# labicon/dp-ilqr

Hardware: AMD Instinct MI355X
Metric: ilqr_subproblems_per_sec (higher is better)
Workload: dtype f64; 1 GPU; cfg2: batches of 1024 independent 5-agent DoubleIntDynamics4D iLQR sub-problems per GPU per step, T=50, scripts/analysis.py scenario distribution, tol=1e-3, n_lqr_iter=50; 2468 steps = 2527232 distinct seeds per GPU, window of 6144 in flight; 1 repetition(s) of the job on disjoint seeds, the median is reported; batch_per_gpu=1024, window=6144, n_x=20, n_u=10, horizon=50, parallelism=single GPU

## Files before the change

### dpilqr_amd/csrc/riccati_mfma.hpp

```cpp
#pragma once
#include <hip/hip_runtime.h>

#include <type_traits>

#include "tiles.hpp"
#include "wave_util.hpp"

namespace dpilqr {

typedef double v4d __attribute__((ext_vector_type(4)));

template <int N, int M, int FUSED = 0, bool HELP = false>
struct MfmaCfg {
    static constexpr int NM = N + M;
    static constexpr int NP = N + 1;
    static constexpr int MK = round_up(M, 4);
    static constexpr int LAB = round_up(NM, 2);
    static constexpr int LT = LAB;
    static constexpr int LP = round_up(NP, 2);
    static constexpr int LQ = LP;
    static constexpr int LG = round_up(M + NP, 2);
    static constexpr int LK = LP;
    static constexpr int LM = N;
    static constexpr int KROWS = MK + 2;
    static constexpr int T_NM = (NM + 15) / 16, T_NP = (NP + 15) / 16, T_N = (N + 15) / 16, T_M = (M + 15) / 16;
    static constexpr int LTB = LP;
    static constexpr int F_KA = N / 4, F_NP = F_KA * (F_KA - 1) / 2;
    static constexpr int F_W = FUSED == 2 ? F_KA : 1;
    static constexpr int oFG = N * LQ, oFH = oFG + 2 * F_NP, oFD = oFH + 4 * F_NP, oFQQ = oFD + 4 * F_KA, oFRR = oFQQ + 16 * F_W,
                         oFXf = oFRR + 4 * F_W, oFL = oFXf + N, oFA = oFL + round_up(NM, 2),
                         szF1 = round_up(oFA + (FUSED == 2 ? 4 * F_KA : 0), 2);
    static constexpr int oFflag = szF1;
    static constexpr int FB = HELP ? round_up(szF1 + 2 - oFG, 2) : 0;
    static constexpr int szF = HELP ? round_up(oFG + 2 * FB, 2) : szF1;
    static constexpr int szR1 = FUSED ? szF : round_up(N * LAB > N * LQ ? N * LAB : N * LQ, 2);
    static constexpr int szT0 = N * LT > KROWS * LK + MK * N ? N * LT : KROWS * LK + MK * N;
    static constexpr int szT1 = szT0 > NM * LTB ? szT0 : NM * LTB;
    static constexpr int szR2 = round_up(szT1 > N * LP ? szT1 : N * LP, 2);
    static constexpr int szG0 = MK * LG + round_up(N, 2);
    static constexpr int szG = round_up(szG0 > NP * LM ? szG0 : NP * LM, 2);
    static constexpr int oAB = 0;
    static constexpr int oQ = 0;
    static constexpr int oT = oAB + szR1;
    static constexpr int oK = oT;
    static constexpr int oT3 = oK + KROWS * LK;
    static constexpr int oP = oT;
    static constexpr int oG = oT + szR2;
    static constexpr int oQx = oG + MK * LG;
    static constexpr int oEnd0 = oG + szG;
    static constexpr bool TEAM_TAIL = HELP && (NP > 16) && (NP <= 32) && (M <= 16);
    static constexpr int oA2 = oEnd0;
    static constexpr int oEnd = oEnd0 + (TEAM_TAIL ? round_up(NP * LM, 2) : 0);
    static constexpr int total = round_up(oEnd + 8, 2);
    static constexpr bool supported = (N % 4 == 0) && (M % 2 == 0) && (N + M + 1 <= 64) && (total * 8 <= 40 * 1024);
    static constexpr int AB_PAIRS = N * NM / 2;
    static constexpr int AB_ROUNDS = (AB_PAIRS + 63) / 64;
};

template <int N, int M, int PNS>
struct InprodCfg {
    static constexpr int PNC = PNS == 6 ? 3 : (PNS == 12 ? 4 : 2);
    static constexpr int KA = PNS > 0 ? ((N / (PNS > 0 ? PNS : 1)) < (M / PNC) ? (N / (PNS > 0 ? PNS : 1)) : (M / PNC)) : 0;
    static constexpr int NPR = KA * (KA - 1) / 2, NPR1 = NPR > 0 ? NPR : 1;
    static constexpr int oLxx = 0;
    static constexpr int oLuu = oLxx + N * N;
    static constexpr int oLxu = oLuu + M * M;
    static constexpr int oX = oLxu + round_up(N + M, 2);
    static constexpr int oE = oX + round_up(N, 2);
    static constexpr int oU = oE + round_up(N, 2);
    static constexpr int oXf = oU + round_up(M, 2);
    static constexpr int oGp = oXf + round_up(N, 2);
    static constexpr int oHp = oGp + round_up(3 * NPR1, 2);
    static constexpr int oQQ = oHp + round_up(9 * NPR1, 2);
    static constexpr int oRR = oQQ + round_up(KA * PNS * PNS, 2);
    static constexpr int oPair = round_up(oRR + KA * PNC * PNC, 2);
    static constexpr int total = PNS > 0 ? round_up(oPair + (NPR1 + 1) / 2, 2) : 0;
};

template <int L>
__device__ __forceinline__ double dpp_fmac_row(double acc, double a, double b) {
    asm("s_nop 1\n\tv_fmac_f64_dpp %0, %1, %2 row_newbcast:%3 row_mask:0xf bank_mask:0xf" : "+v"(acc) : "v"(a), "v"(b), "n"(L));
    return acc;
}
template <int L>
__device__ __forceinline__ double dpp_fmac_row_nn(double acc, double a, double b) {
    asm volatile("v_fmac_f64_dpp %0, %1, %2 row_newbcast:%3 row_mask:0xf bank_mask:0xf" : "+v"(acc) : "v"(a), "v"(b), "n"(L));
    return acc;
}
template <int L>
__device__ __forceinline__ double dpp_mov_row(double a) {
    double r;
    asm("s_nop 1\n\tv_mov_b64_dpp %0, %1 row_newbcast:%2 row_mask:0xf bank_mask:0xf" : "=v"(r) : "v"(a), "n"(L));
    return r;
}
#define DPILQR_ROW_SWITCH(FN, ...)                                                                                  \
    switch (l) {                                                                                                    \
    case 0: return FN<0>(__VA_ARGS__); case 1: return FN<1>(__VA_ARGS__); case 2: return FN<2>(__VA_ARGS__);        \
    case 3: return FN<3>(__VA_ARGS__); case 4: return FN<4>(__VA_ARGS__); case 5: return FN<5>(__VA_ARGS__);        \
    case 6: return FN<6>(__VA_ARGS__); case 7: return FN<7>(__VA_ARGS__); case 8: return FN<8>(__VA_ARGS__);        \
    case 9: return FN<9>(__VA_ARGS__); case 10: return FN<10>(__VA_ARGS__); case 11: return FN<11>(__VA_ARGS__);    \
    case 12: return FN<12>(__VA_ARGS__); case 13: return FN<13>(__VA_ARGS__); case 14: return FN<14>(__VA_ARGS__);  \
    default: return FN<15>(__VA_ARGS__);                                                                            \
    }
__device__ __forceinline__ double fmac_row(double acc, double a, double b, int l) { DPILQR_ROW_SWITCH(dpp_fmac_row, acc, a, b) }
__device__ __forceinline__ double fmac_row_nn(double acc, double a, double b, int l) { DPILQR_ROW_SWITCH(dpp_fmac_row_nn, acc, a, b) }
__device__ __forceinline__ double mov_row(double a, int l) { DPILQR_ROW_SWITCH(dpp_mov_row, a) }

__device__ __forceinline__ v4d mfma_f64(double a, double b, v4d c) {
    return __builtin_amdgcn_mfma_f64_16x16x4f64(a, b, c, 0, 0, 0);
}

template <int TI, int TJ, int KLEN, int LDX, int LDY>
__device__ __forceinline__ void mfma_product(const double* __restrict__ px, const double* __restrict__ py,
                                             v4d (&acc)[TI][TJ]) {
    static_assert(KLEN % 4 == 0, "reduction length must be padded to a multiple of 4");
#pragma unroll
    for (int ks = 0; ks < KLEN / 4; ++ks) {
        double a[TI], b[TJ];
#pragma unroll
        for (int it = 0; it < TI; ++it) a[it] = px[ks * 4 * LDX + 16 * it];
#pragma unroll
        for (int jt = 0; jt < TJ; ++jt) b[jt] = py[ks * 4 * LDY + 16 * jt];
#pragma unroll
        for (int it = 0; it < TI; ++it)
#pragma unroll
            for (int jt = 0; jt < TJ; ++jt) acc[it][jt] = mfma_f64(a[it], b[jt], acc[it][jt]);
    }
}

template <int TI, int TJ>
__device__ __forceinline__ void zero_tiles(v4d (&acc)[TI][TJ]) {
#pragma unroll
    for (int it = 0; it < TI; ++it)
#pragma unroll
        for (int jt = 0; jt < TJ; ++jt) acc[it][jt] = v4d{0.0, 0.0, 0.0, 0.0};
}

template <typename F>
__device__ __forceinline__ void for_rows(int row0, int lo, int hi, int g, bool col_ok, F&& f) {
#pragma unroll
    for (int v = 0; v < 4; ++v) {
        const int r = row0 + 4 * v;
        if (r + 3 < lo || r >= hi) continue;
        const bool inside = (r >= lo) && (r + 3 < hi);
        if (col_ok && (inside || (r + g >= lo && r + g < hi))) f(v, r - lo);
    }
}

template <typename F>
__device__ __forceinline__ void for_rows_p(int row0, int lo, int hi, int g, bool col_ok, F&& f) {
#pragma unroll
    for (int v = 0; v < 4; ++v) {
        const int r = row0 + 4 * v;
        if (r + 3 < lo || r >= hi) continue;
        const bool inside = (r >= lo) && (r + 3 < hi);
        f(v, r - lo, col_ok && (inside || (r + g >= lo && r + g < hi)));
    }
}

template <bool SEARCH, int M, bool ROWLU, bool KEEPINV = true, bool BATCH = false>
__device__ __forceinline__ void lu_eliminate(double (&v_io)[M], double (&invd)[KEEPINV ? M : 1], int& sing, int* swaps = nullptr) {
    double v[M];
#pragma unroll
    for (int r = 0; r < M; ++r) v[r] = v_io[r];
#pragma unroll
    for (int kk = 0; kk < M; ++kk) {
        if constexpr (SEARCH) {
            double mx = 0.0;
#pragma unroll
            for (int r = kk + 1; r < M; ++r) mx = fmax(mx, fabs(v[r]));
            const unsigned long long need = __builtin_amdgcn_ballot_w64(mx > fabs(v[kk]));
            if ((need >> kk) & 1ull) {
                if (swaps) *swaps += 1;
                int piv = kk;
                double best = fabs(v[kk]);
#pragma unroll
                for (int r = kk + 1; r < M; ++r) {
                    const double av = fabs(v[r]);
                    piv = (av > best) ? r : piv;
                    best = fmax(best, av);
                }
                piv = __builtin_amdgcn_readlane(piv, kk);
                asm volatile("" ::: "memory");
#pragma unroll
                for (int r = kk + 1; r < M; ++r)
                    if (r == piv) {
                        asm volatile("" ::: "memory");
                        const double tv = v[r]; v[r] = v[kk]; v[kk] = tv;
                    }
            }
        }
        const double pv = ROWLU ? mov_row(v[kk], kk) : readlane_f64(v[kk], kk);
        if (SEARCH && pv == 0.0) sing = 1;
        double inv = __builtin_amdgcn_rcp(pv);
        inv = fma(fma(-pv, inv, 1.0), inv, inv);
        inv = fma(fma(-pv, inv, 1.0), inv, inv);
        if constexpr (KEEPINV) invd[kk] = inv;
        if constexpr (ROWLU) {
            const double ninv = -inv;
            if constexpr (!BATCH) {
#pragma unroll
                for (int r = kk + 1; r < M; ++r) v[r] = fmac_row(v[r], v[r] * ninv, v[kk], kk);
            } else {
#pragma unroll
            for (int r0 = kk + 1; r0 < M; r0 += 3) {
                double tm[3];
#pragma unroll
                for (int q = 0; q < 3; ++q)
                    if (r0 + q < M) { tm[q] = v[r0 + q] * ninv; asm volatile("" : "+v"(tm[q])); }
                if (r0 + 2 >= M) asm volatile("s_nop 1");
#pragma unroll
                for (int q = 0; q < 3; ++q)
                    if (r0 + q < M) { v[r0 + q] = fmac_row_nn(v[r0 + q], tm[q], v[kk], kk); asm volatile("" : "+v"(v[r0 + q])); }
            }
            }
        } else {
#pragma unroll
            for (int r = kk + 1; r < M; ++r) {
                const double l = readlane_f64(v[r], kk) * inv;
                v[r] = fma(-l, v[kk], v[r]);
            }
        }
    }
#pragma unroll
    for (int r = 0; r < M; ++r) v_io[r] = v[r];
}

__device__ __forceinline__ void wave_barrier_all() { asm volatile("s_waitcnt lgkmcnt(0)\n\ts_barrier" ::: "memory"); }

template <bool ON>
__device__ __forceinline__ int phase_lane(int lane) {
    if constexpr (ON) asm volatile("" : "+v"(lane));
    return lane;
}

struct FusedArgs {
    dpilqr_batch_desc D;
    const double* X;
    const double* U;
    int no_decoupled = 0;
};

template <int N, int M, int WAVES, int NS, int NC, int FUSED, bool PAD = false, bool HELP = false, int PNS = 0>
__device__ __forceinline__ void riccati_mfma_sweep(
    int B, int T, const double* __restrict__ tiles, const double* __restrict__ mu_arr, double* __restrict__ Kout,
    double* __restrict__ dout, int32_t* __restrict__ singular, const int32_t* __restrict__ items,
    const int32_t* __restrict__ n_items, int gains_by_item, int n_cus, FusedArgs F, int n_rec = N, int m_rec = M) {
    using C = MfmaCfg<N, M, FUSED, HELP>;
    static_assert(!FUSED || (NS == 4 && NC == 2), "the fused variants are written for the four-state family's blocks");
    static_assert(!HELP || (FUSED != 0 && WAVES == 4), "the helper wavefront serves the fused forms at one item per SIMD");
    static_assert(!PAD || (NS == 0 && FUSED == 0), "padding while loading is written for the dense record-fed form");
    static_assert(PNS == 0 || (NS == 0 && FUSED == 0 && !HELP), "in-sweep production builds on the dense form (padded, or of the exact size: n_rec = N, m_rec = M)");
    constexpr bool INP = PNS > 0;
    using IC = InprodCfg<N, M, PNS>;
    constexpr bool FGEN = (FUSED == 2);
    constexpr int NM = C::NM, NP = C::NP, MK = C::MK, LAB = C::LAB, LT = C::LT, LP = C::LP, LQ = C::LQ, LG = C::LG;
    constexpr int LK = C::LK, LM = C::LM, T_NM = C::T_NM, T_NP = C::T_NP, T_N = C::T_N, T_M = C::T_M;
    const int wave_all = threadIdx.x >> 6;
    const bool helper = HELP && wave_all >= 4;
    const int wave = HELP ? (wave_all & 3) : wave_all;
    const int n = n_items ? *n_items : B;
    constexpr int LPR = WAVES / 4;
    const int per_layer = 4 * n_cus;
    const int layers = (n + per_layer - 1) / per_layer;
    const int rounds = (layers + LPR - 1) / LPR;
    const int round = (int)blockIdx.x / n_cus, cu = (int)blockIdx.x - round * n_cus;
    if (round >= rounds) return;
    const int lo = layers / rounds, extra = layers - lo * rounds;
    const int my_layers = lo + (round < extra ? 1 : 0);
    const int first_layer = round * lo + min(round, extra);
    if (wave >= 4 * my_layers) return;
    const int slot = (first_layer + (wave >> 2)) * per_layer + (wave & 3) * n_cus + cu;
    if (slot >= n) return;
    const int b = items ? items[slot] : slot;
    if (b >= B) return;
    const int64_t gslot = gains_by_item ? b : slot;
    const int lane0 = threadIdx.x & 63;
    const TileLayout L(PAD ? n_rec : N, PAD ? m_rec : M);

    extern __shared__ __attribute__((aligned(16))) double lds_all[];
    double* lds = lds_all + wave * (C::total + IC::total);
    double* sAB = lds + C::oAB;
    double* sT = lds + C::oT;
    double* sK = lds + C::oK;
    double* sT3 = lds + C::oT3;
    double* sP = lds + C::oP;
    double* sQ = lds + C::oQ;
    double* sG = lds + C::oG;
    double* sQx = lds + C::oQx;
    double* sMt = C::TEAM_TAIL ? lds + C::oA2 : sG;

    const double mu = mu_arr[b];
    const double f_radius = FUSED ? F.D.radius[(int64_t)b * F.D.radius_bstride] : 0.0;
    const double* base = (FUSED || INP) ? nullptr : tiles + (int64_t)slot * (T + 1) * L.stride;
    int sing = 0;
    unsigned long long* const stamps = g_stamp_buf;
    unsigned long long t_start = 0;
    if (stamps) t_start = __builtin_amdgcn_s_memrealtime();

    constexpr bool ROWLU = (M < 16) && (4 * (16 - M) >= NP);
    constexpr int K_PAIRS = M * N / 2, K_ROUNDS = (K_PAIRS + 63) / 64;
    constexpr bool BD = NS > 0;
    constexpr int KA = BD ? N / (BD ? NS : 1) : 1, LPA = 64 / KA, NSC = NS + NC;
    constexpr int CPL = 2 * ((NP + 2 * LPA - 1) / (2 * LPA));
    constexpr int RPL = (NM + LPA - 1) / LPA;
    constexpr int LTB = C::LTB;
    static_assert(!BD || (NS % 2 == 0 && NC % 2 == 0 && N % 2 == 0 && M % 2 == 0 && CPL == 2),
                  "block-diagonal variant: 16-byte vector accesses need even block sizes");
    v2d nbL[RPL][NSC / 2 > 0 ? NSC / 2 : 1];
    v2d nbX[NSC / 2 > 0 ? NSC / 2 : 1];
    constexpr bool LATE_L = BD && (WAVES == 12);
    v2d nAB[C::AB_ROUNDS];
    double nL[T_NM][T_NM][4];
    double nLxu[T_NM][4];
    constexpr bool REMAT = (WAVES == 12) || (PAD && N >= 20);
    v2d pf[2];
    bool f_prox = false;
    double lvc[FUSED ? RPL : 1][FUSED ? NSC : 1];
    int lv_h[FUSED ? RPL : 1];
    bool lv_neg[FUSED ? RPL : 1];
    int t_cur = T;
    if constexpr (HELP) {
        if (helper) {
            const int lane = lane0;
            wave_barrier_all();
            {
                t_cur = T - 1;
#include "riccati_mfma_lane.inc"
                fused_prefetch(T - 1);
            }
            for (int t = T - 1; t >= 0; --t) {
                t_cur = t;
#include "riccati_mfma_lane.inc"
                __builtin_amdgcn_s_waitcnt(0x0F70);
                fused_step_data(t, nullptr);
                if (lane == 0) sFflag[0] = f_prox ? 1.0 : 0.0;
                if (t > 0) fused_prefetch(t - 1);
                if constexpr (C::TEAM_TAIL) {
                    if (t < T - 1) {
                        wave_barrier_all();
                        constexpr int IT = 1;
#include "riccati_mfma_team_tail.inc"
                    }
                }
                wave_barrier_all();
            }
            if constexpr (C::TEAM_TAIL) {
                t_cur = 0;
#include "riccati_mfma_lane.inc"
                wave_barrier_all();
                constexpr int IT = 1;
#include "riccati_mfma_team_tail.inc"
                wave_barrier_all();
            }
            return;
        }
    }
#include "riccati_mfma_inprod.inc"
    {
    const int lane = lane0;
    for (int e = lane; e < C::total + IC::total; e += 64) lds[e] = 0.0;
    DPILQR_LDS_FENCE();
    if constexpr (INP) {
        inp_constants();
        inp_prefetch(T);
        inp_produce(T, true);
        for (int e = lane; e < N * N; e += 64) {
            const int i = e / N, j = e - i * N;
            sP[i * LP + j] = sLxx[e];
        }
        for (int i = lane; i < N; i += 64) sP[i * LP + N] = sLxu[i];
        DPILQR_LDS_FENCE();
        inp_lxx_blocks(false, true);
        inp_prefetch(T - 1);
    } else if constexpr (!FUSED) {
        const double* rec = base + (int64_t)T * L.stride;
        for (int e = lane; e < N * N; e += 64) {
            const int i = e / N, j = e - i * N;
            if constexpr (PAD) {
                const double val = rec[L.oLxx + min(i, n_rec - 1) * n_rec + min(j, n_rec - 1)];
                sP[i * LP + j] = (i < n_rec && j < n_rec) ? val : 0.0;
            } else {
            sP[i * LP + j] = rec[L.oLxx + e];
            }
        }
        for (int i = lane; i < N; i += 64) {
            const double val = rec[L.oLx + (PAD ? min(i, n_rec - 1) : i)];
            sP[i * LP + N] = (!PAD || i < n_rec) ? val : 0.0;
        }
    }

#include "riccati_mfma_lane.inc"
    if constexpr (FUSED) {
        const ItemParams IP = item_params(F.D, b);
        if constexpr (FGEN) {
            for (int e = lane; e < 16 * FKA; e += 64) {
                const int a = e >> 4, q = e & 15;
                sFQQ[e] = IP.Q[16 * a + q] + IP.Q[16 * a + (q & 3) * 4 + (q >> 2)];
            }
            for (int e = lane; e < 4 * FKA; e += 64) {
                const int a = e >> 2, q = e & 3;
                sFRR[e] = IP.R[4 * a + q] + IP.R[4 * a + (q & 1) * 2 + (q >> 1)];
            }
        } else {
        if (lane < 16) sFQQ[lane] = IP.Q[lane] + IP.Q[(lane & 3) * 4 + (lane >> 2)];
        if (lane < 4) sFRR[lane] = IP.R[lane] + IP.R[(lane & 1) * 2 + (lane >> 1)];
        }
        for (int e = lane; e < N; e += 64) sFXf[e] = IP.xf[e];
        DPILQR_LDS_FENCE();
        if constexpr (HELP) wave_barrier_all();
        fused_prefetch(T);
        __builtin_amdgcn_s_waitcnt(0x0F70);
        fused_step_data(T, IP.Qf);
        for (int e = lane; e < N * N; e += 64) {
            const int i = e / N, j = e - i * N, ai = i >> 2, li = i & 3, aj = j >> 2, lj = j & 3;
            double val = 0.0;
            if (ai == aj) {
                const double* Qfa = IP.Qf + (FGEN ? 16 * ai : 0);
                val = F.D.w_ref * (Qfa[li * 4 + lj] + Qfa[lj * 4 + li]);
            }
            if (FKA > 1 && li < 2 && lj < 2 && f_prox) {
                double acc = 0.0;
                if (ai == aj) acc = sFD[ai * 4 + li * 2 + lj];
                else acc += -sFH[((ai < aj) ? pair_index(ai, aj, FKA) : pair_index(aj, ai, FKA)) * 4 + li * 2 + lj];
                val += F.D.w_prox * acc;
            }
            sP[i * LP + j] = val;
        }
        for (int j = lane; j < N; j += 64) sP[j * LP + N] = sFL[j];
        DPILQR_LDS_FENCE();
        if constexpr (!HELP) fused_prefetch(T - 1);
    } else if constexpr (INP) {
    } else {
    prefetch_ab(T - 1);
    if constexpr (BD) {
        prefetch_bd_x(T - 1);
        if constexpr (!LATE_L) prefetch_bd_l(T - 1);
    } else {
        prefetch_lxu(T - 1);
        prefetch_l(T - 1);
    }
    }
    __builtin_amdgcn_s_waitcnt(0x0F70);
    }

    int t_first = T - 1;
    if constexpr (FUSED == 1 && !HELP) {
        if (!F.no_decoupled && !f_prox) {
            const int lane = lane0;
            static_assert(32 * KA <= C::szG, "the prologue's exchange area must fit the G region");
            const ItemParams IP = item_params(F.D, b);
            const int da = min(lane >> 3, KA - 1), dc = min(lane & 7, 4);
            const bool dst = dc < 4;
            const int dcol = dst ? 4 * da + dc : N;
            const double fdt = F.D.dt, wref = F.D.w_ref;
            double* sX = sG + 32 * da;
            double Pc[4];
#pragma unroll
            for (int l = 0; l < 4; ++l) Pc[l] = sP[(4 * da + l) * LP + dcol];
            const int cq = dc & 3, cr = dc & 1;
            const double inf_ = __builtin_inf();
            double chk0 = fabs(mu) + fabs(fdt);
#pragma unroll
            for (int l = 0; l < 4; ++l) chk0 = chk0 + fabs(Pc[l]);
            if (__builtin_amdgcn_ballot_w64(!(chk0 < inf_)) == 0ull) {
                DPILQR_LDS_FENCE();
                for (int e = lane; e < C::szR2; e += 64) sT[e] = 0.0;
                static_assert(20 <= N * LQ, "the prologue's constants must fit the Q_xx region");
                if (lane < 16) sQ[lane] = wref * (IP.Q[(lane & 3) * 4 + (lane >> 2)] + IP.Q[(lane >> 2) * 4 + (lane & 3)]);
                else if (lane < 20) sQ[lane] = wref * (IP.R[(lane & 1) * 2 + ((lane >> 1) & 1)] + IP.R[((lane >> 1) & 1) * 2 + (lane & 1)]);
                DPILQR_LDS_FENCE();
                int t = T - 1;
                for (; t >= 0; --t) {
                    t_cur = t;
                    const int lane = phase_lane<REMAT>(lane0);
#include "riccati_mfma_lane.inc"
                    fused_step_data(t, nullptr);
                    if (f_prox) break;
                    fused_prefetch(t > 0 ? t - 1 : 0);
                    double tt[6];
                    tt[0] = Pc[0];
                    tt[1] = Pc[1];
                    tt[2] = fdt * Pc[0] + Pc[2];
                    tt[3] = fdt * Pc[1] + Pc[3];
                    tt[4] = fdt * Pc[2];
                    tt[5] = fdt * Pc[3];
                    tt[4] = fma(mu, (dst && dc == 2) ? fdt : 0.0, tt[4]);
                    tt[5] = fma(mu, (dst && dc == 3) ? fdt : 0.0, tt[5]);
                    if (dc < 2) {
#pragma unroll
                        for (int r = 0; r < 6; ++r) sX[2 * r + dc] = tt[r];
                    }
                    DPILQR_LDS_FENCE();
                    double qc[4], gc[2], quu[2];
                    {
                        double tu[6], lx[6], lq[4], lr[2];
                        {
                            const v2d q0 = *reinterpret_cast<const v2d*>(sQ + 4 * cq), q1 = *reinterpret_cast<const v2d*>(sQ + 4 * cq + 2),
                                      r0 = *reinterpret_cast<const v2d*>(sQ + 16 + 2 * cr);
                            lq[0] = q0.x; lq[1] = q0.y; lq[2] = q1.x; lq[3] = q1.y; lr[0] = r0.x; lr[1] = r0.y;
                        }
#pragma unroll
                        for (int r = 0; r < 6; ++r) tu[r] = sX[2 * r + cr];
#pragma unroll
                        for (int r = 0; r < 4; ++r) lx[r] = sFL[4 * da + r];
                        lx[4] = sFL[N + 2 * da]; lx[5] = sFL[N + 2 * da + 1];
#pragma unroll
                        for (int r = 0; r < 6; ++r) {
                            const double o = (dc < 2) ? tt[r] : tu[r] * fdt + tt[r];
                            const double qv = (r < 4 ? lq[r] : 0.0) + o;
                            const double v = dst ? qv : lx[r] + tt[r];
                            if (r < 4) qc[r] = v; else gc[r - 4] = v;
                        }
#pragma unroll
                        for (int a = 0; a < 2; ++a) quu[a] = lr[a] + tt[4 + a] * fdt;
                    }
                    DPILQR_LDS_FENCE();
                    if (dc == 2 || dc == 3) { sX[12 + cr] = quu[0]; sX[14 + cr] = quu[1]; }
                    DPILQR_LDS_FENCE();
                    const double u00 = sX[12], u01 = sX[13], u10 = sX[14], u11 = sX[15];
                    bool ok;
                    {
                        const double cs0 = (0.0 + fabs(u00)) + fabs(u10), cs1 = (0.0 + fabs(u01)) + fabs(u11);
                        const double dg0 = fabs(u00), dg1 = fabs(u11);
                        ok = (dg0 * (1.0 - 0x1p-20) > cs0 - dg0) && (dg1 * (1.0 - 0x1p-20) > cs1 - dg1);
                    }
                    double inv0 = __builtin_amdgcn_rcp(u00);
                    inv0 = fma(fma(-u00, inv0, 1.0), inv0, inv0);
                    inv0 = fma(fma(-u00, inv0, 1.0), inv0, inv0);
                    const double tm = u10 * (-inv0);
                    const double w11 = fma(tm, u01, u11), g1 = fma(tm, gc[0], gc[1]);
                    double inv1 = __builtin_amdgcn_rcp(w11);
                    inv1 = fma(fma(-w11, inv1, 1.0), inv1, inv1);
                    inv1 = fma(fma(-w11, inv1, 1.0), inv1, inv1);
                    double kc[2];
                    kc[1] = -(g1 * inv1);
                    kc[0] = -(fma(u01, kc[1], gc[0]) * inv0);
                    ok = ok && u00 != 0.0 && w11 != 0.0;
                    const double t30 = fma(u10, kc[1], fma(u00, kc[0], 0.0)), t31 = fma(u11, kc[1], fma(u01, kc[0], 0.0));
                    DPILQR_LDS_FENCE();
                    if (dst) {
                        *reinterpret_cast<v2d*>(sX + 6 * dc) = v2d{t30, t31};
                        *reinterpret_cast<v2d*>(sX + 6 * dc + 2) = v2d{kc[0], kc[1]};
                        *reinterpret_cast<v2d*>(sX + 6 * dc + 4) = v2d{gc[0], gc[1]};
                    }
                    DPILQR_LDS_FENCE();
                    double vc[4];
#pragma unroll
                    for (int i = 0; i < 4; ++i) {
                        const v2d e0 = *reinterpret_cast<const v2d*>(sX + 6 * i), e1 = *reinterpret_cast<const v2d*>(sX + 6 * i + 2),
                                  e2 = *reinterpret_cast<const v2d*>(sX + 6 * i + 4);
                        const double a1 = fma(e0.y, kc[1], fma(e0.x, kc[0], 0.0));
                        const double a2 = fma(e1.y, gc[1], fma(e1.x, gc[0], 0.0));
                        const double a2t = fma(kc[1], e2.y, fma(kc[0], e2.x, 0.0));
                        vc[i] = ((qc[i] + a1) + a2) + a2t;
                    }
                    DPILQR_LDS_FENCE();
                    if (dst) {
#pragma unroll
                        for (int i = 0; i < 4; ++i) sX[4 * i + dc] = vc[i];
                    }
                    DPILQR_LDS_FENCE();
                    double pn[4];
                    {
                        const v2d w0 = *reinterpret_cast<const v2d*>(sX + 4 * cq), w1 = *reinterpret_cast<const v2d*>(sX + 4 * cq + 2);
                        pn[0] = dst ? 0.5 * (vc[0] + w0.x) : vc[0];
                        pn[1] = dst ? 0.5 * (vc[1] + w0.y) : vc[1];
                        pn[2] = dst ? 0.5 * (vc[2] + w1.x) : vc[2];
                        pn[3] = dst ? 0.5 * (vc[3] + w1.y) : vc[3];
                    }
                    DPILQR_LDS_FENCE();
                    double chk = fabs(u00) + fabs(u01);
                    chk = chk + fabs(u10); chk = chk + fabs(u11); chk = chk + fabs(w11); chk = chk + fabs(inv0); chk = chk + fabs(inv1);
                    chk = chk + fabs(gc[0]); chk = chk + fabs(gc[1]); chk = chk + fabs(g1); chk = chk + fabs(kc[0]); chk = chk + fabs(kc[1]);
                    chk = chk + fabs(t30); chk = chk + fabs(t31);
#pragma unroll
                    for (int i = 0; i < 4; ++i) chk = chk + fabs(pn[i]);
                    ok = ok && chk < inf_;
                    if (__builtin_amdgcn_ballot_w64(!ok) != 0ull) {
                        fused_prefetch(t);
                        break;
                    }
#pragma unroll
                    for (int l = 0; l < 4; ++l) Pc[l] = pn[l];
                    sK[(2 * da) * LK + dcol] = kc[0];
                    sK[(2 * da + 1) * LK + dcol] = kc[1];
                    DPILQR_LDS_FENCE();
                    double* Kt = Kout + (gslot * T + t) * M * N;
                    double* dt_ = dout + (gslot * T + t) * M;
#pragma unroll
                    for (int q = 0; q < K_ROUNDS; ++q) store_v2d_nt(Kt + k_out[q], *reinterpret_cast<const v2d*>(sK + k_in[q]));
                    store_f64_nt(dt_ + d_idx, sK[d_idx * LK + N]);
                    DPILQR_LDS_FENCE();
                }
                t_first = t;
                for (int e = lane; e < 32 * KA; e += 64) sG[e] = 0.0;
                if (lane < 20) sQ[lane] = 0.0;
                for (int e = lane; e < C::szR2; e += 64) sT[e] = 0.0;
                DPILQR_LDS_FENCE();
#pragma unroll
                for (int l = 0; l < 4; ++l) sP[(4 * da + l) * LP + dcol] = Pc[l];
                DPILQR_LDS_FENCE();
            }
        }
    }

    if constexpr (FUSED) {
        const ItemParams IP = item_params(F.D, b);
        constexpr int FKA_ = C::F_KA;
        const int ag_ = min(lane0 / LPA, KA - 1), sub2_ = min(lane0 - (lane0 / LPA) * LPA, (NM - 1) / RPL);
#pragma unroll
        for (int r = 0; r < RPL; ++r) {
#pragma unroll
            for (int c = 0; c < NSC; ++c) lvc[r][c] = 0.0;
            lv_h[r] = -1; lv_neg[r] = false;
            const int ip = min(RPL * sub2_ + r, NM - 1);
            if (ip < N) {
                const int ar = ip >> 2, li = ip & 3;
                if (ar == ag_) {
                    const double* Qa = IP.Q + (FGEN ? 16 * ag_ : 0);
#pragma unroll
                    for (int c = 0; c < NS; ++c) lvc[r][c] = F.D.w_ref * (Qa[li * 4 + c] + Qa[c * 4 + li]);
                }
                if (FKA_ > 1 && li < 2) {
                    lv_neg[r] = ar != ag_;
                    lv_h[r] = (ar == ag_) ? (C::oFD - C::oFH) + ag_ * 4 + li * 2
                                          : ((ar < ag_) ? pair_index(ar, ag_, FKA_) : pair_index(ag_, ar, FKA_)) * 4 + li * 2;
                }
            } else {
                const int a = ip - N;
                if ((a >> 1) == ag_) {
                    const double* Ra = IP.R + (FGEN ? 4 * ag_ : 0);
                    lvc[r][NS] = F.D.w_ref * (Ra[(a & 1) * 2] + Ra[a & 1]);
                    lvc[r][NS + 1] = F.D.w_ref * (Ra[(a & 1) * 2 + 1] + Ra[2 + (a & 1)]);
                }
            }
        }
    }

#ifdef DPILQR_PHASE_STAMPS
    unsigned long long ph[8] = {0, 0, 0, 0, 0, 0, 0, 0}, ph_t = __builtin_amdgcn_s_memtime();
#define MPHASE(i) { asm volatile("s_waitcnt lgkmcnt(0)" ::: "memory"); const unsigned long long now_ = __builtin_amdgcn_s_memtime(); ph[i] += now_ - ph_t; ph_t = now_; }
#elif defined(DPILQR_PHASE_MARKS)
#define MPHASE(i) asm volatile("; ==== end of phase " #i);
#else
#define MPHASE(i)
#endif
    for (int t = t_first; t >= 0; --t) {
        const int tn = t > 0 ? t - 1 : 0;
        t_cur = t;
        {
        const int lane = phase_lane<REMAT>(lane0);
#include "riccati_mfma_lane.inc"
        if constexpr (HELP) {
            wave_barrier_all();
            f_prox = __builtin_amdgcn_readfirstlane((int)(sFflag[0] != 0.0)) != 0;
        } else if constexpr (FUSED) {
            fused_step_data(t, nullptr);
            fused_prefetch(tn);
        } else if constexpr (INP) {
            inp_produce(t, false);
            inp_prefetch(tn);
        } else {
#pragma unroll
        for (int q = 0; q < C::AB_ROUNDS; ++q) *reinterpret_cast<v2d*>(ab_dst[q]) = nAB[q];
        DPILQR_LDS_FENCE();
        if constexpr (LATE_L) prefetch_bd_l(t);
        prefetch_ab(tn);
        }
        MPHASE(0)

        __builtin_amdgcn_s_setprio(1);
        if constexpr (FUSED) {
            const double fdt = F.D.dt;
            double acc[NSC][CPL], pr[NS][CPL];
#pragma unroll
            for (int l = 0; l < NS; ++l) {
                const v2d v = *reinterpret_cast<const v2d*>(bP + l * LP);
                pr[l][0] = v.x; pr[l][1] = v.y;
            }
            double fa[4] = {0.0, 0.0, 0.0, 0.0};
            if constexpr (FGEN) {
                const v2d a0 = *reinterpret_cast<const v2d*>(sFA + 4 * ag), a1 = *reinterpret_cast<const v2d*>(sFA + 4 * ag + 2);
                fa[0] = a0.x; fa[1] = a0.y; fa[2] = a1.x; fa[3] = a1.y;
            }
#pragma unroll
            for (int c = 0; c < CPL; ++c) {
                acc[0][c] = pr[0][c];
                acc[1][c] = pr[1][c];
                if constexpr (FGEN) {
                    acc[2][c] = fma(fa[1], pr[1][c], fa[0] * pr[0][c]) + pr[2][c];
                    acc[3][c] = fma(fa[3], pr[1][c], fa[2] * pr[0][c]) + pr[3][c];
                } else {
                acc[2][c] = fdt * pr[0][c] + pr[2][c];
                acc[3][c] = fdt * pr[1][c] + pr[3][c];
                }
                acc[4][c] = fdt * pr[2][c];
                acc[5][c] = fdt * pr[3][c];
#pragma unroll
                for (int q = 0; q < NC; ++q) acc[NS + q][c] = fma(mu, (j0 + c == 4 * ag + 2 + q) ? fdt : 0.0, acc[NS + q][c]);
            }
#pragma unroll
            for (int r = 0; r < NS; ++r) *reinterpret_cast<v2d*>(bTa + r * LTB) = v2d{acc[r][0], acc[r][1]};
#pragma unroll
            for (int r = 0; r < NC; ++r) *reinterpret_cast<v2d*>(bTb + r * LTB) = v2d{acc[NS + r][0], acc[NS + r][1]};
            if (bPcol) {
#pragma unroll
                for (int r = 0; r < NS; ++r) sQx[NS * ag + r] = sFL[NS * ag + r] + acc[r][0];
#pragma unroll
                for (int r = 0; r < NC; ++r) sG[(NC * ag + r) * LG + M + N] = sFL[N + NC * ag + r] + acc[NS + r][0];
            }
        } else if constexpr (BD) {
            double acc[NSC][CPL];
#pragma unroll
            for (int l = 0; l < NS; ++l) {
                double ab[NSC], pr[CPL];
#pragma unroll
                for (int q = 0; q < NS / 2; ++q) {
                    const v2d v = *reinterpret_cast<const v2d*>(bABa + l * LAB + 2 * q);
                    ab[2 * q] = v.x; ab[2 * q + 1] = v.y;
                }
#pragma unroll
                for (int q = 0; q < NC / 2; ++q) {
                    const v2d v = *reinterpret_cast<const v2d*>(bABb + l * LAB + 2 * q);
                    ab[NS + 2 * q] = v.x; ab[NS + 2 * q + 1] = v.y;
                }
                {
                    const v2d v = *reinterpret_cast<const v2d*>(bP + l * LP);
                    pr[0] = v.x; pr[1] = v.y;
                }
#pragma unroll
                for (int r = 0; r < NSC; ++r)
#pragma unroll
                    for (int c = 0; c < CPL; ++c) acc[r][c] = (l == 0) ? ab[r] * pr[c] : fma(ab[r], pr[c], acc[r][c]);
            }
#pragma unroll
            for (int c = 0; c < CPL; ++c)
#pragma unroll
                for (int q = 0; q < NC / 2; ++q) {
                    const v2d v = *reinterpret_cast<const v2d*>(bBmu[c] + 2 * q);
                    acc[NS + 2 * q][c] = fma(mu, bMuOn[c] ? v.x : 0.0, acc[NS + 2 * q][c]);
                    acc[NS + 2 * q + 1][c] = fma(mu, bMuOn[c] ? v.y : 0.0, acc[NS + 2 * q + 1][c]);
                }
#pragma unroll
            for (int r = 0; r < NS; ++r) *reinterpret_cast<v2d*>(bTa + r * LTB) = v2d{acc[r][0], acc[r][1]};
#pragma unroll
            for (int r = 0; r < NC; ++r) *reinterpret_cast<v2d*>(bTb + r * LTB) = v2d{acc[NS + r][0], acc[NS + r][1]};
            if (bPcol) {
#pragma unroll
                for (int r = 0; r < NS; ++r) sQx[NS * ag + r] = ((r & 1) ? nbX[r / 2].y : nbX[r / 2].x) + acc[r][0];
#pragma unroll
                for (int r = 0; r < NC; ++r)
                    sG[(NC * ag + r) * LG + M + N] = ((r & 1) ? nbX[NS / 2 + r / 2].y : nbX[NS / 2 + r / 2].x) + acc[NS + r][0];
            }
        } else {
            v4d acc[T_NM][T_NP];
            zero_tiles(acc);
            mfma_product<T_NM, T_NP, N, LAB, LP>(pAB, pP, acc);
#pragma unroll
            for (int it = 0; it < T_NM; ++it)
#pragma unroll
                for (int jt = 0; jt < T_NP; ++jt) {
                    for_rows(16 * it, 0, N, g, colN[jt], [&](int v, int r) { dTt[16 * jt * LT + r] = acc[it][jt][v]; });
                    for_rows(16 * it, N, NM, g, colN[jt], [&](int v, int r) {
                        dTt[16 * jt * LT + N + r] = fma(mu, dBt[16 * jt * LAB + N + r], acc[it][jt][v]);
                    });
                    if (16 * jt <= N && N < 16 * jt + 16) {
                        for_rows(16 * it, 0, N, g, colP[jt], [&](int v, int r) {
                            sQx[g + r] = (INP ? sLxu[g + r] : nLxu[it][v]) + acc[it][jt][v];
                        });
                        for_rows(16 * it, N, NM, g, colP[jt], [&](int v, int r) {
                            dG[M + N + r * LG] = (INP ? sLxu[N + g + r] : nLxu[it][v]) + acc[it][jt][v];
                        });
                    }
                }
        }
        DPILQR_LDS_FENCE();
        if constexpr (!BD && !FUSED && !INP) prefetch_lxu(tn);
        MPHASE(1)
        }
        {
        const int lane = phase_lane<REMAT>(lane0);
#include "riccati_mfma_lane.inc"

        if constexpr (FUSED) {
            const double fdt = F.D.dt, wp = F.D.w_prox;
            double fa2[4] = {0.0, 0.0, 0.0, 0.0};
            if constexpr (FGEN) {
                const v2d a0 = *reinterpret_cast<const v2d*>(sFA + 4 * ag), a1 = *reinterpret_cast<const v2d*>(sFA + 4 * ag + 2);
                fa2[0] = a0.x; fa2[1] = a0.y; fa2[2] = a1.x; fa2[3] = a1.y;
            }
            v2d hh[RPL];
            const bool with_h = FKA > 1 && f_prox;
            if (with_h) {
#pragma unroll
                for (int r = 0; r < RPL; ++r) hh[r] = *reinterpret_cast<const v2d*>(sFH + max(lv_h[r], 0));
            }
#pragma unroll
            for (int r = 0; r < RPL; ++r) {
                double tv[NS], acc[NSC], lv[NSC];
#pragma unroll
                for (int q = 0; q < NS / 2; ++q) {
                    const v2d v = *reinterpret_cast<const v2d*>(bT2[r] + 2 * q);
                    tv[2 * q] = v.x; tv[2 * q + 1] = v.y;
                }
                acc[0] = tv[0]; acc[1] = tv[1];
                if constexpr (FGEN) {
                    acc[2] = fma(tv[1], fa2[1], tv[0] * fa2[0]) + tv[2];
                    acc[3] = fma(tv[1], fa2[3], tv[0] * fa2[2]) + tv[3];
                } else {
                acc[2] = tv[0] * fdt + tv[2]; acc[3] = tv[1] * fdt + tv[3];
                }
                acc[4] = tv[2] * fdt; acc[5] = tv[3] * fdt;
#pragma unroll
                for (int c = 0; c < NSC; ++c) lv[c] = lvc[r][c];
                if (with_h) {
                    const bool on = lv_h[r] >= 0;
                    const double l0 = lv[0] + wp * (lv_neg[r] ? -hh[r].x : hh[r].x), l1 = lv[1] + wp * (lv_neg[r] ? -hh[r].y : hh[r].y);
                    lv[0] = on ? l0 : lv[0];
                    lv[1] = on ? l1 : lv[1];
                }
#pragma unroll
                for (int q = 0; q < NS / 2; ++q)
                    *reinterpret_cast<v2d*>(bDa[r] + 2 * q) = v2d{lv[2 * q] + acc[2 * q], lv[2 * q + 1] + acc[2 * q + 1]};
                *reinterpret_cast<v2d*>(bDb[r]) = v2d{lv[NS] + acc[NS], lv[NS + 1] + acc[NS + 1]};
            }
        } else if constexpr (BD) {
            double acc[RPL][NSC];
            double tv[RPL][NS];
            {
#pragma unroll
                for (int r = 0; r < RPL; ++r)
#pragma unroll
                    for (int q = 0; q < NS / 2; ++q) {
                        const v2d v = *reinterpret_cast<const v2d*>(bT2[r] + 2 * q);
                        tv[r][2 * q] = v.x; tv[r][2 * q + 1] = v.y;
                    }
            }
#pragma unroll
            for (int l = 0; l < NS; ++l) {
                double ab[NSC];
#pragma unroll
                for (int q = 0; q < NS / 2; ++q) {
                    const v2d v = *reinterpret_cast<const v2d*>(bABa + l * LAB + 2 * q);
                    ab[2 * q] = v.x; ab[2 * q + 1] = v.y;
                }
#pragma unroll
                for (int q = 0; q < NC / 2; ++q) {
                    const v2d v = *reinterpret_cast<const v2d*>(bABb + l * LAB + 2 * q);
                    ab[NS + 2 * q] = v.x; ab[NS + 2 * q + 1] = v.y;
                }
#pragma unroll
                for (int r = 0; r < RPL; ++r) {
                    const double tvl = tv[r][l];
#pragma unroll
                    for (int c = 0; c < NSC; ++c) acc[r][c] = (l == 0) ? tvl * ab[c] : fma(tvl, ab[c], acc[r][c]);
                }
            }
#pragma unroll
            for (int r = 0; r < RPL; ++r) {
#pragma unroll
                for (int q = 0; q < NS / 2; ++q)
                    *reinterpret_cast<v2d*>(bDa[r] + 2 * q) = v2d{nbL[r][q].x + acc[r][2 * q], nbL[r][q].y + acc[r][2 * q + 1]};
#pragma unroll
                for (int q = 0; q < NC / 2; ++q)
                    *reinterpret_cast<v2d*>(bDb[r] + 2 * q) =
                        v2d{nbL[r][NS / 2 + q].x + acc[r][NS + 2 * q], nbL[r][NS / 2 + q].y + acc[r][NS + 2 * q + 1]};
            }
        } else {
            v4d acc[T_NM][T_NM];
            zero_tiles(acc);
            mfma_product<T_NM, T_NM, N, LT, LAB>(pT, pAB, acc);
#pragma unroll
            for (int it = 0; it < T_NM; ++it)
#pragma unroll
                for (int jt = 0; jt < T_NM; ++jt) {
                    if constexpr (INP) {
                        const int j = 16 * jt + c16;
                        for_rows(16 * it, 0, N, g, colN[jt], [&](int v, int r) {
                            dQ[16 * jt + r * LQ] = sLxx[(g + r) * N + j] + acc[it][jt][v];
                        });
                        for_rows(16 * it, N, NM, g, colNM[jt], [&](int v, int r) {
                            const double luu = sLuu[(g + r) * M + max(j - N, 0)];
                            dG[colG[jt] + r * LG] = (j >= N ? luu : 0.0) + acc[it][jt][v];
                        });
                    } else {
                    for_rows(16 * it, 0, N, g, colN[jt], [&](int v, int r) { dQ[16 * jt + r * LQ] = nL[it][jt][v] + acc[it][jt][v]; });
                    for_rows(16 * it, N, NM, g, colNM[jt], [&](int v, int r) { dG[colG[jt] + r * LG] = nL[it][jt][v] + acc[it][jt][v]; });
                    }
                }
        }
        DPILQR_LDS_FENCE();
        if (lane < N) sQ[lane * LQ + N] = sQx[lane];
        if constexpr (FUSED || INP) {} else if constexpr (BD) { prefetch_bd_x(tn); if constexpr (!LATE_L) prefetch_bd_l(tn); } else prefetch_l(tn);
        for (int e = lane; e < (C::KROWS - M) * LK; e += 64) sK[M * LK + e] = 0.0;
        MPHASE(2)
        }
        {
        const int lane = phase_lane<REMAT>(lane0);
#include "riccati_mfma_lane.inc"

        {
            const int col = s3_col;
            double v[M], invd[M];
#pragma unroll
            for (int r = 0; r < M; ++r) v[r] = sG[r * LG + col];
            double colsum = 0.0;
#pragma unroll
            for (int r = 0; r < M; ++r) colsum = colsum + fabs(v[r]);
            const double dg = fabs(sG[s3_dg]);
            const bool dominant = !s3_lhs || dg * (1.0 - 0x1p-20) > colsum - dg;
            const bool no_swaps = __builtin_amdgcn_ballot_w64(!dominant) == 0ull;
            constexpr bool LUB = ROWLU && (WAVES == 4);
            if (no_swaps) lu_eliminate<false, M, ROWLU, true, LUB>(v, invd, sing); else lu_eliminate<true, M, ROWLU, true, LUB>(v, invd, sing);
            if constexpr (ROWLU) {
                double nv[M];
#pragma unroll
                for (int r = M - 1; r >= 0; --r) {
                    double s = v[r];
#pragma unroll
                    for (int c = r + 1; c < M; ++c) s = fmac_row_nn(s, v[r], nv[c], c);
                    nv[r] = -(s * invd[r]);
                }
#pragma unroll
                for (int r = 0; r < M; ++r) v[r] = -nv[r];
            } else {
#pragma unroll
                for (int r = M - 1; r >= 0; --r) {
                    double s = v[r];
#pragma unroll
                    for (int c = r + 1; c < M; ++c) s = fma(-readlane_f64(v[r], c), v[c], s);
                    v[r] = s * invd[r];
                }
            }
#pragma unroll
            for (int a = 0; a < M; ++a) s3_k[a * LK] = -v[a];
        }
        DPILQR_LDS_FENCE();
        if constexpr (PAD) {
            double* Kt = Kout + (gslot * T + t) * m_rec * n_rec;
            double* dt_ = dout + (gslot * T + t) * m_rec;
            const double* krow = sK + min(lane, N - 1);
            double kv[M];
#pragma unroll
            for (int a = 0; a < M; ++a) kv[a] = krow[a * LK];
#pragma unroll
            for (int a = 0; a < M; ++a)
                if (a < m_rec && lane < n_rec) store_f64_nt(Kt + a * n_rec + lane, kv[a]);
            if (lane < m_rec) store_f64_nt(dt_ + lane, sK[lane * LK + N]);
        } else {
            double* Kt = Kout + (gslot * T + t) * M * N;
            double* dt_ = dout + (gslot * T + t) * M;
#pragma unroll
            for (int q = 0; q < K_ROUNDS; ++q) store_v2d_nt(Kt + k_out[q], *reinterpret_cast<const v2d*>(sK + k_in[q]));
            store_f64_nt(dt_ + d_idx, sK[d_idx * LK + N]);
        }
        DPILQR_LDS_FENCE();
        MPHASE(3)
        }
        {
        const int lane = phase_lane<REMAT>(lane0);
#include "riccati_mfma_lane.inc"

        __builtin_amdgcn_s_setprio(0);
        if constexpr (C::TEAM_TAIL) {
            wave_barrier_all();
            constexpr int IT = 0;
#include "riccati_mfma_team_tail.inc"
            if (t == 0) wave_barrier_all();
        } else {
        constexpr bool T3R = (T_M == 1) && (T_N == T_NP) && (WAVES != 12);
        v4d t3[T_M][T_N];
        zero_tiles(t3);
        mfma_product<T_M, T_N, MK, LG, LK>(pGuu, pK, t3);
        if constexpr (!T3R) {
#pragma unroll
            for (int it = 0; it < T_M; ++it)
#pragma unroll
                for (int jt = 0; jt < T_N; ++jt)
                    for_rows(16 * it, 0, M, g, colN[jt], [&](int v, int r) { dT3[16 * jt + r * N] = t3[it][jt][v]; });
            DPILQR_LDS_FENCE();
        }
        MPHASE(4)

        {
            double vb[T_NP][T_NP][4];
            v4d a1[T_NP][T_NP], a2[T_NP][T_NP];
            zero_tiles(a1);
            zero_tiles(a2);
            if constexpr (T3R) {
#pragma unroll
                for (int ks = 0; ks < MK / 4; ++ks) {
                    double b[T_NP];
#pragma unroll
                    for (int jt = 0; jt < T_NP; ++jt) b[jt] = pK[ks * 4 * LK + 16 * jt];
#pragma unroll
                    for (int it = 0; it < T_NP; ++it)
#pragma unroll
                        for (int jt = 0; jt < T_NP; ++jt) a1[it][jt] = mfma_f64(t3[0][it][ks], b[jt], a1[it][jt]);
                }
            } else {
                mfma_product<T_NP, T_NP, MK, N, LK>(pT3, pK, a1);
            }
            mfma_product<T_NP, T_NP, MK, LK, LG>(pK, pGux, a2);
#pragma unroll
            for (int it = 0; it < T_NP; ++it)
#pragma unroll
                for (int jt = 0; jt < T_NP; ++jt)
                    for_rows(16 * it, 0, NP, g, colN[jt], [&](int v, int r) { dMt[16 * jt + r * LM] = a2[it][jt][v]; });
            DPILQR_LDS_FENCE();
#pragma unroll
            for (int it = 0; it < T_NP; ++it)
#pragma unroll
                for (int jt = 0; jt < T_NP; ++jt) {
#pragma unroll
                    for (int v = 0; v < 4; ++v) vb[it][jt][v] = 0.0;
                    for_rows_p(16 * it, 0, N, g, colLE[jt], [&](int v, int r, bool ok) {
                        const double q = *(ok ? dQ + 16 * jt + r * LQ : sP), mt = *(ok ? dMtT + 16 * jt * LM + r : sP);
                        vb[it][jt][v] = ((q + a1[it][jt][v]) + a2[it][jt][v]) + mt;
                    });
                }
            DPILQR_LDS_FENCE();
#pragma unroll
            for (int it = 0; it < T_NP; ++it)
#pragma unroll
                for (int jt = 0; jt < T_NP; ++jt)
                    for_rows(16 * it, 0, N, g, colLE[jt], [&](int v, int r) { dP[16 * jt + r * LP] = vb[it][jt][v]; });
            DPILQR_LDS_FENCE();
#pragma unroll
            for (int it = 0; it < T_NP; ++it)
#pragma unroll
                for (int jt = 0; jt < T_NP; ++jt) {
                    for_rows_p(16 * it, 0, N, g, colN[jt], [&](int v, int r, bool ok) {
                        vb[it][jt][v] = 0.5 * (vb[it][jt][v] + *(ok ? dPt + 16 * jt * LP + r : sP));
                    });
                }
            DPILQR_LDS_FENCE();
#pragma unroll
            for (int it = 0; it < T_NP; ++it)
#pragma unroll
                for (int jt = 0; jt < T_NP; ++jt)
                    for_rows(16 * it, 0, N, g, colN[jt], [&](int v, int r) { dP[16 * jt + r * LP] = vb[it][jt][v]; });
        }
        }
        DPILQR_LDS_FENCE();
        MPHASE(5)
        }
    }
    if (singular && sing && lane0 == 0) singular[b] = 1;
    if (stamps && lane0 == 0) {
        unsigned hw_id, xcc_id;
        asm volatile("s_getreg_b32 %0, hwreg(HW_REG_HW_ID)" : "=s"(hw_id));
        asm volatile("s_getreg_b32 %0, hwreg(HW_REG_XCC_ID)" : "=s"(xcc_id));
        stamps[4 * slot + 0] = t_start;
        stamps[4 * slot + 1] = __builtin_amdgcn_s_memrealtime();
        stamps[4 * slot + 2] = hw_id;
        stamps[4 * slot + 3] = xcc_id;
#ifdef DPILQR_PHASE_STAMPS
        for (int i = 0; i < 7; ++i) stamps[4 * B + 8 * slot + i] = ph[i];
#endif
    }
}

template <int N, int M, int WAVES, int NS, int NC, bool FUSED = false>
__global__ __launch_bounds__(64 * WAVES, WAVES / 4) void k_riccati_mfma(
    int B, int T, const double* __restrict__ tiles, const double* __restrict__ mu_arr, double* __restrict__ Kout,
    double* __restrict__ dout, int32_t* __restrict__ singular, const int32_t* __restrict__ items,
    const int32_t* __restrict__ n_items, int gains_by_item, int n_cus, FusedArgs F) {
    riccati_mfma_sweep<N, M, WAVES, NS, NC, (FUSED ? 1 : 0)>(B, T, tiles, mu_arr, Kout, dout, singular, items, n_items, gains_by_item, n_cus, F);
}

template <int N, int M, int FUSED>
__global__ __launch_bounds__(512, 2) void k_riccati_mfma_team(
    int B, int T, const double* __restrict__ mu_arr, double* __restrict__ Kout, double* __restrict__ dout,
    int32_t* __restrict__ singular, const int32_t* __restrict__ items, const int32_t* __restrict__ n_items, int gains_by_item,
    int n_cus, FusedArgs F) {
    riccati_mfma_sweep<N, M, 4, 4, 2, FUSED, false, true>(B, T, nullptr, mu_arr, Kout, dout, singular, items, n_items, gains_by_item,
                                                          n_cus, F);
}

template <int N, int M, int WAVES>
__global__ __launch_bounds__(64 * WAVES, WAVES / 4) void k_riccati_mfma_pad(
    int B, int T, const double* __restrict__ tiles, const double* __restrict__ mu_arr, double* __restrict__ Kout,
    double* __restrict__ dout, int32_t* __restrict__ singular, const int32_t* __restrict__ items,
    const int32_t* __restrict__ n_items, int gains_by_item, int n_cus, int n_rec, int m_rec) {
    riccati_mfma_sweep<N, M, WAVES, 0, 0, 0, true>(B, T, tiles, mu_arr, Kout, dout, singular, items, n_items, gains_by_item, n_cus,
                                                   FusedArgs{}, n_rec, m_rec);
}

template <int N, int M, int WAVES, int PNS, bool PAD>
__global__ __launch_bounds__(64 * WAVES, WAVES / 4) void k_riccati_mfma_inprod(
    int B, int T, const double* __restrict__ mu_arr, double* __restrict__ Kout, double* __restrict__ dout,
    int32_t* __restrict__ singular, const int32_t* __restrict__ items, const int32_t* __restrict__ n_items, int gains_by_item,
    int n_cus, FusedArgs F, int n_rec, int m_rec) {
    riccati_mfma_sweep<N, M, WAVES, 0, 0, 0, PAD, false, PNS>(B, T, nullptr, mu_arr, Kout, dout, singular, items, n_items,
                                                              gains_by_item, n_cus, F, PAD ? n_rec : N, PAD ? m_rec : M);
}

template <int N, int M, int WAVES>
__global__ __launch_bounds__(64 * WAVES, WAVES / 4) void k_riccati_mfma_general(
    int B, int T, const double* __restrict__ mu_arr, double* __restrict__ Kout, double* __restrict__ dout,
    int32_t* __restrict__ singular, const int32_t* __restrict__ items, const int32_t* __restrict__ n_items, int gains_by_item,
    int n_cus, FusedArgs F) {
    riccati_mfma_sweep<N, M, WAVES, 4, 2, 2>(B, T, nullptr, mu_arr, Kout, dout, singular, items, n_items, gains_by_item, n_cus, F);
}

}
```

Measured before the change: 1.031 million subproblems/s.

## Streamline fused Riccati prologue step with DPP exchange and fewer LDS fences

Reworks the decoupled double-integrator prologue loop of the fused Riccati kernel. A row-shift DPP replaces the LDS round-trip used to share tt values between lanes. The Q constants are laid out so each lane reads its l-values with 16-byte loads through precomputed pointers. Branchy stores become unconditional writes to dummy slots, the K stores are merged into an existing fence region with pointers decremented each step, lane setup is hoisted out of the loop, and the finiteness check is shortened. This cuts LDS traffic and barriers per step, but the shorter check and removed sT reset could change how non-finite values are handled.

```diff
diff --git a/dpilqr_amd/csrc/riccati_mfma.hpp b/dpilqr_amd/csrc/riccati_mfma.hpp
--- a/dpilqr_amd/csrc/riccati_mfma.hpp
+++ b/dpilqr_amd/csrc/riccati_mfma.hpp
@@ -87,6 +87,11 @@
     asm volatile("v_fmac_f64_dpp %0, %1, %2 row_newbcast:%3 row_mask:0xf bank_mask:0xf" : "+v"(acc) : "v"(a), "v"(b), "n"(L));
     return acc;
 }
+__device__ __forceinline__ double dpp_row_shr2(double v) {
+    const int lo = __builtin_amdgcn_update_dpp(0, __double2loint(v), 0x112, 0xf, 0xf, true);
+    const int hi = __builtin_amdgcn_update_dpp(0, __double2hiint(v), 0x112, 0xf, 0xf, true);
+    return __hiloint2double(hi, lo);
+}
 template <int L>
 __device__ __forceinline__ double dpp_mov_row(double a) {
     double r;
@@ -459,6 +464,14 @@
 #pragma unroll
             for (int l = 0; l < 4; ++l) Pc[l] = sP[(4 * da + l) * LP + dcol];
             const int cq = dc & 3, cr = dc & 1;
+            const bool dmid = dc == 2 || dc == 3;
+            const double mu4 = dc == 2 ? fdt : 0.0, mu5 = dc == 3 ? fdt : 0.0;
+            static_assert(C::oFL % 2 == 0 && N % 2 == 0 && C::oG % 2 == 0, "16-byte reads of the prologue's l-values");
+            const double* const lvA = dst ? sQ + 6 * dc : lds + C::oQ + C::oFL + 4 * da;
+            const double* const lvB = dst ? sQ + 6 * dc + 4 : lds + C::oQ + C::oFL + N + 2 * da;
+            double* const x4 = sX + 6 * dc;
+            double* const x5 = sX + (dst ? dc : 16);
+            double* const x2 = sX + (dmid ? 12 : 28) + cr;
             const double inf_ = __builtin_inf();
             double chk0 = fabs(mu) + fabs(fdt);
 #pragma unroll
@@ -466,15 +479,24 @@
             if (__builtin_amdgcn_ballot_w64(!(chk0 < inf_)) == 0ull) {
                 DPILQR_LDS_FENCE();
                 for (int e = lane; e < C::szR2; e += 64) sT[e] = 0.0;
-                static_assert(20 <= N * LQ, "the prologue's constants must fit the Q_xx region");
-                if (lane < 16) sQ[lane] = wref * (IP.Q[(lane & 3) * 4 + (lane >> 2)] + IP.Q[(lane >> 2) * 4 + (lane & 3)]);
-                else if (lane < 20) sQ[lane] = wref * (IP.R[(lane & 1) * 2 + ((lane >> 1) & 1)] + IP.R[((lane >> 1) & 1) * 2 + (lane & 1)]);
+                static_assert(24 <= N * LQ, "the prologue's constants must fit the Q_xx region");
+                if (lane < 24) {
+                    const int c = lane / 6, r = lane - 6 * c, r3 = min(r, 3);
+                    const double qv = wref * (IP.Q[r3 * 4 + c] + IP.Q[c * 4 + r3]);
+                    sQ[lane] = r < 4 ? qv : 0.0;
+                }
                 DPILQR_LDS_FENCE();
+                const double lr0 = wref * (IP.R[cr] + IP.R[cr * 2]), lr1 = wref * (IP.R[2 + cr] + IP.R[cr * 2 + 1]);
+#include "riccati_mfma_lane.inc"
+                double* Kt = Kout + (gslot * T + (T - 1)) * M * N;
+                double* dt_ = dout + (gslot * T + (T - 1)) * M + d_idx;
+                const double* const kd_in = sK + d_idx * LK + N;
+                double* const k_st0 = sK + (2 * da) * LK + dcol;
                 int t = T - 1;
                 for (; t >= 0; --t) {
-                    t_cur = t;
-                    const int lane = phase_lane<REMAT>(lane0);
-#include "riccati_mfma_lane.inc"
+#ifdef DPILQR_PHASE_MARKS
+                    asm volatile("; ==== prologue step: begin");
+#endif
                     fused_step_data(t, nullptr);
                     if (f_prox) break;
                     fused_prefetch(t > 0 ? t - 1 : 0);
@@ -485,40 +507,33 @@
                     tt[3] = fdt * Pc[1] + Pc[3];
                     tt[4] = fdt * Pc[2];
                     tt[5] = fdt * Pc[3];
-                    tt[4] = fma(mu, (dst && dc == 2) ? fdt : 0.0, tt[4]);
-                    tt[5] = fma(mu, (dst && dc == 3) ? fdt : 0.0, tt[5]);
-                    if (dc < 2) {
-#pragma unroll
-                        for (int r = 0; r < 6; ++r) sX[2 * r + dc] = tt[r];
+                    tt[4] = fma(mu, mu4, tt[4]);
+                    tt[5] = fma(mu, mu5, tt[5]);
+                    double qc[4], gc[2], quu[2];
+                    {
+                        double tu[6], o[6];
+#pragma unroll
+                        for (int r = 0; r < 6; ++r) tu[r] = dpp_row_shr2(tt[r]);
+                        const v2d l0 = *reinterpret_cast<const v2d*>(lvA), l1 = *reinterpret_cast<const v2d*>(lvA + 2),
+                                  l2 = *reinterpret_cast<const v2d*>(lvB);
+#pragma unroll
+                        for (int r = 0; r < 6; ++r) o[r] = tt[r];
+                        if (dmid) {
+#pragma unroll
+                            for (int r = 0; r < 6; ++r) o[r] = tu[r] * fdt + tt[r];
+                        }
+                        qc[0] = l0.x + o[0]; qc[1] = l0.y + o[1]; qc[2] = l1.x + o[2]; qc[3] = l1.y + o[3];
+                        gc[0] = l2.x + o[4]; gc[1] = l2.y + o[5];
+                        quu[0] = lr0 + tt[4] * fdt; quu[1] = lr1 + tt[5] * fdt;
                     }
                     DPILQR_LDS_FENCE();
-                    double qc[4], gc[2], quu[2];
+                    x2[0] = quu[0]; x2[2] = quu[1];
+                    DPILQR_LDS_FENCE();
+                    double u00, u01, u10, u11;
                     {
-                        double tu[6], lx[6], lq[4], lr[2];
-                        {
-                            const v2d q0 = *reinterpret_cast<const v2d*>(sQ + 4 * cq), q1 = *reinterpret_cast<const v2d*>(sQ + 4 * cq + 2),
-                                      r0 = *reinterpret_cast<const v2d*>(sQ + 16 + 2 * cr);
-                            lq[0] = q0.x; lq[1] = q0.y; lq[2] = q1.x; lq[3] = q1.y; lr[0] = r0.x; lr[1] = r0.y;
-                        }
-#pragma unroll
-                        for (int r = 0; r < 6; ++r) tu[r] = sX[2 * r + cr];
-#pragma unroll
-                        for (int r = 0; r < 4; ++r) lx[r] = sFL[4 * da + r];
-                        lx[4] = sFL[N + 2 * da]; lx[5] = sFL[N + 2 * da + 1];
-#pragma unroll
-                        for (int r = 0; r < 6; ++r) {
-                            const double o = (dc < 2) ? tt[r] : tu[r] * fdt + tt[r];
-                            const double qv = (r < 4 ? lq[r] : 0.0) + o;
-                            const double v = dst ? qv : lx[r] + tt[r];
-                            if (r < 4) qc[r] = v; else gc[r - 4] = v;
-                        }
-#pragma unroll
-                        for (int a = 0; a < 2; ++a) quu[a] = lr[a] + tt[4 + a] * fdt;
+                        const v2d ua = *reinterpret_cast<const v2d*>(sX + 12), ub = *reinterpret_cast<const v2d*>(sX + 14);
+                        u00 = ua.x; u01 = ua.y; u10 = ub.x; u11 = ub.y;
                     }
-                    DPILQR_LDS_FENCE();
-                    if (dc == 2 || dc == 3) { sX[12 + cr] = quu[0]; sX[14 + cr] = quu[1]; }
-                    DPILQR_LDS_FENCE();
-                    const double u00 = sX[12], u01 = sX[13], u10 = sX[14], u11 = sX[15];
                     bool ok;
                     {
                         const double cs0 = (0.0 + fabs(u00)) + fabs(u10), cs1 = (0.0 + fabs(u01)) + fabs(u11);
@@ -539,11 +554,11 @@
                     ok = ok && u00 != 0.0 && w11 != 0.0;
                     const double t30 = fma(u10, kc[1], fma(u00, kc[0], 0.0)), t31 = fma(u11, kc[1], fma(u01, kc[0], 0.0));
                     DPILQR_LDS_FENCE();
-                    if (dst) {
-                        *reinterpret_cast<v2d*>(sX + 6 * dc) = v2d{t30, t31};
-                        *reinterpret_cast<v2d*>(sX + 6 * dc + 2) = v2d{kc[0], kc[1]};
-                        *reinterpret_cast<v2d*>(sX + 6 * dc + 4) = v2d{gc[0], gc[1]};
-                    }
+                    *reinterpret_cast<v2d*>(x4) = v2d{t30, t31};
+                    *reinterpret_cast<v2d*>(x4 + 2) = v2d{kc[0], kc[1]};
+                    *reinterpret_cast<v2d*>(x4 + 4) = v2d{gc[0], gc[1]};
+                    k_st0[0] = kc[0];
+                    k_st0[LK] = kc[1];
                     DPILQR_LDS_FENCE();
                     double vc[4];
 #pragma unroll
@@ -556,10 +571,8 @@
                         vc[i] = ((qc[i] + a1) + a2) + a2t;
                     }
                     DPILQR_LDS_FENCE();
-                    if (dst) {
-#pragma unroll
-                        for (int i = 0; i < 4; ++i) sX[4 * i + dc] = vc[i];
-                    }
+#pragma unroll
+                    for (int i = 0; i < 4; ++i) x5[4 * i] = vc[i];
                     DPILQR_LDS_FENCE();
                     double pn[4];
                     {
@@ -570,10 +583,7 @@
                         pn[3] = dst ? 0.5 * (vc[3] + w1.y) : vc[3];
                     }
                     DPILQR_LDS_FENCE();
-                    double chk = fabs(u00) + fabs(u01);
-                    chk = chk + fabs(u10); chk = chk + fabs(u11); chk = chk + fabs(w11); chk = chk + fabs(inv0); chk = chk + fabs(inv1);
-                    chk = chk + fabs(gc[0]); chk = chk + fabs(gc[1]); chk = chk + fabs(g1); chk = chk + fabs(kc[0]); chk = chk + fabs(kc[1]);
-                    chk = chk + fabs(t30); chk = chk + fabs(t31);
+                    double chk = fabs(t30) + fabs(t31);
 #pragma unroll
                     for (int i = 0; i < 4; ++i) chk = chk + fabs(pn[i]);
                     ok = ok && chk < inf_;
@@ -583,20 +593,21 @@
                     }
 #pragma unroll
                     for (int l = 0; l < 4; ++l) Pc[l] = pn[l];
-                    sK[(2 * da) * LK + dcol] = kc[0];
-                    sK[(2 * da + 1) * LK + dcol] = kc[1];
+#pragma unroll
+                    for (int q = 0; q < K_ROUNDS; ++q) store_v2d_nt(Kt + k_out[q], *reinterpret_cast<const v2d*>(sK + k_in[q]));
+                    store_f64_nt(dt_, *kd_in);
+                    Kt -= M * N;
+                    dt_ -= M;
                     DPILQR_LDS_FENCE();
-                    double* Kt = Kout + (gslot * T + t) * M * N;
-                    double* dt_ = dout + (gslot * T + t) * M;
-#pragma unroll
-                    for (int q = 0; q < K_ROUNDS; ++q) store_v2d_nt(Kt + k_out[q], *reinterpret_cast<const v2d*>(sK + k_in[q]));
-                    store_f64_nt(dt_ + d_idx, sK[d_idx * LK + N]);
-                    DPILQR_LDS_FENCE();
+#ifdef DPILQR_PHASE_MARKS
+                    asm volatile("; ==== prologue step: end");
+#endif
                 }
                 t_first = t;
                 for (int e = lane; e < 32 * KA; e += 64) sG[e] = 0.0;
-                if (lane < 20) sQ[lane] = 0.0;
-                for (int e = lane; e < C::szR2; e += 64) sT[e] = 0.0;
+                if (lane < 24) sQ[lane] = 0.0;
+                k_st0[0] = 0.0;
+                k_st0[LK] = 0.0;
                 DPILQR_LDS_FENCE();
 #pragma unroll
                 for (int l = 0; l < 4; ++l) sP[(4 * da + l) * LP + dcol] = Pc[l];
```

New measurement: 945,100 subproblems/s. 8.3% lower.
